# xtcyclist/hash_join_codes_KNL

Measured on AMD Instinct MI355X. Metric: probe Gtuples/s + % HBM roofline, PHJ |R|=64M join |S|=1G, 1/2/4/8 GPU, higher is better.
Workload: dtype u32

## Files before the change

### hash_join_codes_knl_amd/csrc/hj_internal.hpp

```cpp
#pragma once
#include <hip/hip_runtime.h>
#include <stdint.h>
#include <type_traits>
#include "../../include/hjgpu.h"
#include "compact_layout.hpp"

typedef unsigned long long u64;

constexpr uint32_t HJ_LINE_TUPLES = 16;
constexpr uint32_t HJ_STREAM_UNIT = 256;
constexpr uint32_t HJ_MAX_HEAVY = 128;
struct ScatterConfig { int block, vpt; bool carry; };
struct HjTuning;
ScatterConfig hj_scatter_config(const HjTuning &t, int pass, uint32_t F, bool out_packed);
int hj_scatter_tile(const HjTuning &t, int pass, uint32_t F, bool out_packed);
constexpr int HJ_JOIN_SLICE    = 1 << 16;
constexpr int HJ_JOIN_FILL_GROUPS = 64;
inline size_t hj_join_items_capacity(size_t partitions, size_t outer_rows)
{
    return (partitions + outer_rows / HJ_JOIN_SLICE + 1) * HJ_JOIN_FILL_GROUPS;
}

struct JoinConfig {
    int block, log2slots, batch;
    int slots() const { return 1 << log2slots; }
    int cap() const { return slots() / 2; }
};
const JoinConfig &hj_join_config_big();
bool hj_join_config_built(const JoinConfig &c, bool unique);

struct HjTuning {
    int range_tiles = 0;
    bool dense2 = false;
    bool npj_refhash = false;
    bool no_broadcast = false;
    bool force_chained = false;
    bool scatter_prof = false;
    bool unique = false;
    bool piece_interleave = true;
    bool merged_plan = true;
    int placement = 12;
    int placement_ms = 500;
    bool placement_log = false;
    bool exact_probe_counts = false;
    int probe_slack = 12;
    bool solo = false;
    bool audit = false;
    int hist_min_lds = 0;
    int reserve_cus = 0;
    long long host_batch = -1;
    long long group_from = 300000000, group_inner = 64000000;
    bool group_always = false;
    bool group_device = true;
    int group_slack = 50;
    long long batch_tuples = 0;
    JoinConfig join = {512, 13, 2};
    int scatter_cfg[2][3] = {{0, 0, -1}, {0, 0, -1}};
};
void hj_tuning_from_env(HjTuning *t);
bool hj_tuning_set(HjTuning *t, const char *name, const char *value);
inline const JoinConfig &hj_join_config_of(const HjTuning &t, bool big_tables) { return big_tables ? hj_join_config_big() : t.join; }

struct HjPerDeviceOnce { unsigned char done[64]; };
int hj_allow_dynamic_lds(const void *kernel, int bytes, HjPerDeviceOnce *once);

constexpr uint32_t HJ_MAX_RANGE_ENTRIES = 1u << 24;
constexpr uint32_t HJ_MAX_CHUNKS = 256;
constexpr uint32_t HJ_TICKET_K4 = 0;
constexpr uint32_t HJ_TICKET_K6 = 2 * HJ_MAX_CHUNKS;
constexpr uint32_t HJ_TICKET_MULTI_FILL = 2 * HJ_MAX_CHUNKS + 8;
constexpr uint32_t HJ_TICKET_JOIN = 2 * HJ_MAX_CHUNKS + 10;
constexpr uint32_t HJ_TICKET_JOIN2 = 2 * HJ_MAX_CHUNKS + 12;
constexpr uint32_t HJ_TICKET_JOIN3 = 2 * HJ_MAX_CHUNKS + 14;
constexpr uint32_t HJ_TICKET_WORDS = 2 * HJ_MAX_CHUNKS + 16;
struct Pass1Geom {
    u64 n, part;
#if defined(__HIPCC__)
    __host__ __device__
#endif
    u64 beg(uint32_t c) const { return c >= chunks ? n : part * c; }
    uint32_t chunks;
    uint32_t align;
    uint32_t ranges_per_chunk;
    uint32_t tile;
};
// ... 76 lines not shown
    u64 *final_offsets;
    uint32_t *overflow;
    uint32_t nt_rows;
    uint32_t big_tables;
    uint32_t broadcast;
    uint32_t mode;
    const uint32_t *sentinel;
    uint32_t force_chained;
    uint32_t unique;
    u64 *work_counter2;
    const uint32_t *multi_fill;
    uint32_t resume;
    uint32_t s_pieces;
    uint32_t *build_bits;
    u64 *work_counter3;
};
int hj_launch_build_rows(const JoinArgs &a, const HjTuning &t, int cus, hipStream_t stream);
int hj_launch_build_unmatched(const JoinArgs &a, const HjTuning &t, int cus, hipStream_t stream);

struct PlanArgs {
    const u64 *counts[2];
    u64 n[2];
    u64 chunk_beg[2][9];
    u64 *more[2] = {nullptr, nullptr};
    uint32_t regular[2];
    u64 chunk_part[2];
    u64 *off2[2];
    u64 *end2[2];
    uint32_t pad2;
    u64 *cur2[2];
// ... 46 lines not shown
int hj_launch_plan(const PlanArgs &a, hipStream_t stream);
int hj_launch_claimed_pieces(const u64 *off2, const u64 *end2, const u64 *cur2, uint32_t P, u64 *pieces_beg, u64 *pieces_end, hipStream_t stream);
int hj_launch_claimed_desc(const u64 *claim_cursors, u64 cap1, uint32_t F1, uint32_t F2, uint32_t tile2, uint4 *tdesc, uint32_t tdesc_cap,
                           u64 *total, uint32_t *overflow, hipStream_t stream);
struct BatchPlanArgs {
    const uint32_t *range_counts;
    u64 *range_base;
    u64 *boff;
    u64 *tp2b;
    uint4 *tdesc;
    uint32_t tdesc_cap;
    uint32_t ranges, ranges_per_batch, F1, F2, tile2;
};
int hj_launch_batch_plan(const BatchPlanArgs &a, uint32_t batches, hipStream_t stream);
int hj_launch_scatter(const ScatterArgs &a, const HjTuning &t, int cus, hipStream_t stream);
int hj_launch_join(const JoinArgs &a, const HjTuning &t, int cus, hipStream_t stream);
int hj_launch_exscan(const u64 *in, u64 *out, uint32_t n, hipStream_t stream);
int hj_launch_offsets_to_counts(const u64 *off, u64 *counts, uint32_t P, hipStream_t stream);

template <class F>
inline void hj_with_bool(bool b, F &&f)
{
    if (b) f(std::true_type{});
    else f(std::false_type{});
}

int hj_launch_npj_build(const uint32_t *keys, const uint32_t *vals, size_t n, u64 *table,
                        size_t buckets, uint32_t factor, uint32_t *zero_key_flag,
                        int cus, hipStream_t stream, bool line_hash = false);
struct NpjProbeArgs {
    const uint32_t *keys, *vals;
// ... 104 lines not shown
```

### hash_join_codes_knl_amd/csrc/hjgpu_api.hip

```cpp
#include "hjgpu_ctx.hpp"
#include "hj_device.hpp"

using namespace hjapi;



namespace hjapi {


int fail(hjgpu_ctx *ctx, int status, const char *what, hipError_t e)
{
    if (ctx) {
        if (e != hipSuccess)
            snprintf(ctx->err, sizeof(ctx->err), "%s: %s", what, hipGetErrorString(e));
        else
            snprintf(ctx->err, sizeof(ctx->err), "%s", what);
    }
    return status;
}

static int release(hjgpu_ctx *ctx, void *p)
{
    if (!p) return HJGPU_OK;
    HIPCHK(ctx, hipFree(p));
// ... 157 lines not shown
        m.end2[r] = take((size_t)C * P);
        m.cur2[r] = take((size_t)C * P);
        m.off1[r] = take((size_t)C * F1 + 1);
        m.cur1[r] = take((size_t)C * F1);
        m.tp1[r] = take(C + 1);
        m.seg1[r] = take(C + 1);
        m.tp2[r] = take((size_t)C * F1 + 1);
        m.seg2[r] = take((size_t)F1 + 1);
        m.more[r] = C > 8 ? take(P) : nullptr;
    }
    m.claim_total = take(1);
    m.pieces = take((size_t)4 * P);
    m.slice_prefix = take((size_t)P + 1);
    m.slices = take(P);
    m.item_part = reinterpret_cast<uint32_t *>(take(((size_t)P + items_extra + 2) / 2 + 1));
    for (int r = 0; r < 2; ++r) {
        m.range_counts[r] = reinterpret_cast<uint32_t *>(take((ranges * F1 + 1) / 2));
        m.range_base[r] = take(ranges * F1);
    }
    m.tdesc_cap = tiles2;
    for (int r = 0; r < 2; ++r) m.tdesc[r] = reinterpret_cast<uint4 *>(take(tiles2 * 4));
    m.boff = take(batches * ((size_t)F1 + 1));
    m.tp2b = take(batches * ((size_t)F1 + 1));
    m.tdescb = reinterpret_cast<uint4 *>(take(batches * tdesc_b_cap * 4));
    m.btickets = reinterpret_cast<uint32_t *>(take(batches + 1));
    m.btickets_bytes = (batches + 1) * sizeof(u64);
    m.total_bytes = at * sizeof(u64);
    return m;
}

// ... 664 lines not shown
        ja.slice_prefix = m.slice_prefix; ja.slices = m.slices; ja.item_part = m.item_part;
        ja.P = pl.P; ja.chunks = road.pad2 ? 1u : pl.C;
        ja.f1 = pl.f1; ja.F1 = pl.F1; ja.f2 = pl.f2; ja.F2 = pl.F2;
        if (o.pre) { ja.f1 = pl.pre_f1; ja.F1 = pl.pre_F1tot; ja.p1_base = pl.pre_base; }
        ja.tf0 = pl.tf0; ja.tf1 = pl.tf1;
        ja.s_align = 0;
        ja.packed = 1;
        ja.big_tables = pl.big_tables ? 1u : 0u;
        ja.unique = pl.first_match ? 1u : 0u;
        ja.mode = pl.mode;
        ja.result = &st->result;
        ja.work_counter = reinterpret_cast<u64 *>(m.tickets + HJ_TICKET_JOIN);
        ja.work_counter2 = reinterpret_cast<u64 *>(m.tickets + HJ_TICKET_JOIN2);
        ja.work_counter3 = reinterpret_cast<u64 *>(m.tickets + HJ_TICKET_JOIN3);
        ja.multi_fill = m.tickets + HJ_TICKET_MULTI_FILL;
        ja.resume = o.grp ? 1u : 0u;
        join_output(ctx, ja, o.out, bs, bl, st);
        if (marks) {
            ja.build_bits = reinterpret_cast<uint32_t *>(ctx->build_bits.p);
            HIPCHK(ctx, hj_zero_async(ja.build_bits, build_bits_bytes(pl, nn[0]), stream));
            if ((!nn[1] || build_rows) && bs && !o.grp) HIPCHK(ctx, hj_fill_async(ctx->final_offsets.p, 0xFFFFFFFFu, (size_t)workers * sizeof(u64), stream));
        }
        if (nn[1]) CHK(hj_launch_join(ja, ctx->tune, ctx->cus, stream));
        if (build_rows) CHK(hj_launch_build_rows(ja, ctx->tune, ctx->cus, stream));
        else if (marks) CHK(hj_launch_build_unmatched(ja, ctx->tune, ctx->cus, stream));
        if (audit) CHK(hj_audit_copy(reinterpret_cast<const u64 *>(&st->result), audit + 4 * 6, 4, stream));
        return HJGPU_OK;
    }
};

}

int phj_enqueue(hjgpu_ctx *ctx, const PhjPlan &pl, const Rel &R, const Rel &S, hipStream_t stream, const EnqueueOpts &o)
{
    CHK(refuse_capture(ctx, stream));
    if (o.grp && (o.pre || o.stages != PHJ_WHOLE || o.inner_ready)) return fail(ctx, HJGPU_EINVAL, "internal: a device-planned group is a whole join on resident columns");
    if ((o.pre != nullptr) != (pl.pre != 0)) return fail(ctx, HJGPU_EINVAL, "internal: plan and relations disagree about pre-partitioning");
    PhjRun run(ctx, pl, R, S, o, stream);
// ... 6 lines not shown
    CHK(run.begin());
    CHK(run.road.merged ? run.partition_merged() : run.partition_in_turn());
    if (hj_mode_marks_build(pl.mode) && (o.pre || o.stages != PHJ_WHOLE)) return fail(ctx, HJGPU_EINVAL, "internal: a join that marks its build rows is a whole join");
    if (run.road.joins) CHK(run.join(bs, bl, workers));
    record(ctx, EV_JOIN, stream);
    if (bs && run.road.joins && !o.grp) CHK(close_gaps(ctx, o.out, workers, bs, run.st, stream, pl.mode));
    record(ctx, EV_GAPS, stream);
    ctx->stats.fanout1 = pl.F1; ctx->stats.fanout2 = pl.F2; ctx->stats.buckets = 0; ctx->stats.batches = run.batches_used;
    ctx->last_algo = 1;
    return HJGPU_OK;
}

static int finish_from(hjgpu_ctx *ctx, const DevState &h, hjgpu_result *result, const hjgpu_output *out)
{
    if (result) *result = h.result;
    if (h.zero_key) return fail(ctx, HJGPU_EZEROKEY, "NPJ: a build key is 0, the empty-bucket sentinel");
    if (h.overflow) return fail(ctx, HJGPU_EOVERFLOW, "materialised output exceeded its capacity");
    if (out && out->d_keys && h.dense != h.result.count && (h.result.count != 0 || h.dense != 0))
        return fail(ctx, HJGPU_EHIP, "internal: dense length != match count after close_gaps");
    return HJGPU_OK;
}

static int read_state(hjgpu_ctx *ctx, DevState &h, hipStream_t stream)
{
    HIPCHK(ctx, hipMemcpyAsync(&h, ctx->state.p, sizeof(DevState), hipMemcpyDeviceToHost, stream));
    HIPCHK(ctx, hipStreamSynchronize(stream));
    return HJGPU_OK;
}

int finish_blocking(hjgpu_ctx *ctx, hjgpu_result *result, const hjgpu_output *out, hipStream_t stream)
// ... 303 lines not shown
        CHK(phj_prepare(ctx, cap_r, cap_s, &prm, 8, &pl, {.plan_inner = plan_inner}));
    } else {
        CHK(phj_prepare(ctx, inner, outer, &prm, 8, &pl));
        if (claimed_probe_allowed(ctx)) CHK(phj_prepare(ctx, inner, outer, &prm, 1, &pl, {.claim_s = true}));
    }
    size_t buckets; uint32_t factor;
    CHK(npj_prepare(ctx, inner, nullptr, &buckets, &factor));
    return HJGPU_OK;
}

static size_t lds_lookup_rows(const HjTuning &tune);
int hjgpu_get_counter(hjgpu_ctx *ctx, const char *name, uint64_t *value)
{
    if (!ctx || !name || !value) return HJGPU_EINVAL;
    if (strcmp(name, "probe_fallbacks") == 0) { *value = ctx->probe_fallbacks; return HJGPU_OK; }
    if (strcmp(name, "probe_exact") == 0) { *value = (ctx->tune.exact_probe_counts || ctx->probe_exact) ? 1u : 0u; return HJGPU_OK; }
    if (strcmp(name, "lookup_lds_rows") == 0) { *value = lds_lookup_rows(ctx->tune); return HJGPU_OK; }
    if (strcmp(name, "compact_ranges") == 0) { *value = hj_compact::ranges_of(ctx->cus); return HJGPU_OK; }
    if (strcmp(name, "compact_chunk_rows") == 0) { *value = hj_compact::CHUNK_ROWS; return HJGPU_OK; }
    return fail(ctx, HJGPU_EINVAL, "unknown counter (probe_fallbacks, probe_exact, lookup_lds_rows, compact_ranges, compact_chunk_rows)");
}

static void fill_reserve(const hjgpu_ctx *ctx, hjgpu_stats *s)
{
    s->ms_reserve = ctx->ms_reserve;
    s->placement_tried = ctx->placement_tried; s->placement_timeboxed = ctx->placement_timeboxed;
    s->placement_fill_ms = ctx->placement_fill_ms; s->placement_search_ms = ctx->placement_search_ms; s->placement_bytes = (uint64_t)ctx->placement_bytes;
}

int hjgpu_get_stats(hjgpu_ctx *ctx, hjgpu_stats *s)
{
    if (!ctx || !s) return HJGPU_EINVAL;
    if (ctx->stats_override) {
        *s = ctx->stats;
        fill_reserve(ctx, s);
// ... 536 lines not shown
        const Rel g_s = {g_sk + pc[g].s0, g_sv + pc[g].s0, pc[g].sn};
        if (pc[g].rn == 0) {
            CHK(broadcast_enqueue(ctx, {g_rk, g_rv, 0}, g_s, prm, vout, stream, nullptr));
        } else {
            CHK(phj_prepare(ctx, pc[g].rn, pc[g].sn, prm, chunks, &pl));
            CHK(phj_enqueue(ctx, pl, {g_rk + pc[g].r0, g_rv + pc[g].r0, pc[g].rn}, g_s, stream, {.out = vout}));
        }
        DevState h;
        CHK(read_state(ctx, h, stream));
        CHK(hjgpu_get_stats(ctx, &one));
        sum.ms_histogram += one.ms_histogram; sum.ms_plan += one.ms_plan; sum.ms_scatter1 += one.ms_scatter1;
        sum.ms_scatter2 += one.ms_scatter2; sum.ms_join += one.ms_join; sum.ms_close_gaps += one.ms_close_gaps;
        sum.fanout1 = one.fanout1; sum.fanout2 = one.fanout2;
        acc.result.count += h.result.count; acc.result.sum_keys += h.result.sum_keys;
        acc.result.sum_outer_vals += h.result.sum_outer_vals; acc.result.sum_inner_vals += h.result.sum_inner_vals;
        if (h.overflow) { acc.overflow = 1; out_on = false; }
        else if (vout) acc.dense += h.dense;
    }
    HIPCHK(ctx, hipMemcpyAsync(ctx->state.p, &acc, sizeof(DevState), hipMemcpyHostToDevice, stream));
    HIPCHK(ctx, hipStreamSynchronize(stream));
    sum.ms_total = sum.ms_scatter0 + sum.ms_histogram + sum.ms_plan + sum.ms_scatter1 + sum.ms_scatter2 + sum.ms_join + sum.ms_close_gaps;
    sum.groups = G;
    ctx->stats = sum;
    ctx->stats_override = true;
    ctx->last_algo = 1;
    return HJGPU_OK;
}

static void grouped_caps(const hjgpu_ctx *ctx, uint32_t G, size_t inner, size_t outer, size_t *cap_r, size_t *cap_s, size_t *plan_inner)
{
// ... 220 lines not shown
```

### hash_join_codes_knl_amd/csrc/hjgpu_ctx.hpp

```cpp
#pragma once
#include <hip/hip_runtime.h>
#include <algorithm>
#include <chrono>
#include <functional>
#include <math.h>
#include <stdio.h>
#include <stdlib.h>
#include <string.h>
#include <thread>
#include <vector>

#include "hj_internal.hpp"


struct DevBuf {
    void *p = nullptr;
    size_t cap = 0;
};

namespace hjapi {
struct Rel { const uint32_t *keys = nullptr, *vals = nullptr; size_t rows = 0; };
}

struct DevState {
    hjgpu_result result;
    u64 block_counter;
    u64 dense;
    u64 work_counter;
    uint32_t overflow;
    uint32_t zero_key;
    uint32_t nmoves;
    uint32_t pad;
    u64 work_counter2;
    uint32_t group_skew;
    uint32_t probe_overflow;
};

enum { EV_BEGIN = 0, EV_S_HIST, EV_S_PLAN, EV_S_SC1, EV_S_SC2, EV_WAITED,
       EV_R_HIST, EV_R_PLAN, EV_R_SC1, EV_R_SC2, EV_JOIN, EV_GAPS, EV_COUNT };


struct hjgpu_ctx {
    int device = 0;
    int cus = 0;
    hipDeviceProp_t prop;
    char err[512];
    DevBuf tmp[8];
    DevBuf meta;
    DevBuf table;
    DevBuf state;
// ... 6 lines not shown
    hjgpu_stats stats;
    int last_algo = -1;
    bool last_lookup = false;
    bool prepared = false;
    size_t prepared_inner = 0, prepared_max_outer = 0;
    unsigned char prepared_plan[128];
    HjTuning tune;
    hipStream_t host_streams[3] = {nullptr, nullptr, nullptr};
    void *host_stage[4] = {nullptr, nullptr, nullptr, nullptr};
    hipEvent_t host_stage_ev[4] = {nullptr, nullptr, nullptr, nullptr};
    hjgpu_output pending_out;
    bool has_pending_out = false;
    bool last_had_output = false;
    uint64_t probe_fallbacks = 0;
    bool probe_exact = false;
    bool rows_plain = false;
    DevBuf grp[4], grp_off;
    bool stats_override = false;
    hipStream_t aux = nullptr;
    hipEvent_t *ev_cur = nullptr;
    std::vector<hipEvent_t> grp_ev;
    uint32_t grp_ev_groups = 0;
    hipEvent_t grp_ev_pass0[3] = {nullptr, nullptr, nullptr};
    struct GroupedCall {
        bool valid = false;
        uint32_t chunks = 1;
        hjapi::Rel R, S;
        bool has_prm = false, has_out = false;
        hjgpu_phj_params prm;
        hjgpu_output out;
// ... 70 lines not shown
    return n < 1 ? 1 : n;
}

inline uint32_t align_of(const void *p) { return (uint32_t)(((uintptr_t)p >> 2) & 3); }

struct MetaLayout {
    u64 *counts[2], *off2[2], *end2[2], *cur2[2], *off1[2], *cur1[2], *tp1[2], *seg1[2], *tp2[2];
    u64 *claim1;
    u64 *claim_total;
    u64 *pieces;
    u64 *seg2[2];
    u64 *more[2];
    u64 *slice_prefix, *slices;
    uint32_t *tickets;
    uint32_t *item_part;
    uint4 *tdesc[2];
    size_t tdesc_cap;
    uint32_t *range_counts[2];
    u64 *range_base[2];
    u64 *boff, *tp2b;
    uint4 *tdescb;
    uint32_t *btickets;
    size_t btickets_bytes;
    size_t counts_bytes;
    size_t total_bytes;
};
MetaLayout carve(void *base, uint32_t C, uint32_t F1, uint32_t P, size_t ranges, size_t items_extra = 0,
                 size_t tiles2 = 0, size_t batches = 0, size_t tdesc_b_cap = 0);
ScatterArgs scatter_pass1(const hjgpu_ctx *ctx, const MetaLayout &m, int r, const Pass1Geom &geom, uint32_t F, uint32_t factor,
                          const uint32_t *kin, const uint32_t *vin, uint32_t *kout, uint32_t *vout);
// ... 92 lines not shown
```

### hash_join_codes_knl_amd/csrc/join_kernels.hip

```cpp
#include "hj_device.hpp"
#include "hj_internal.hpp"
#include "hj_emit.hpp"
#include "hj_lookup.hpp"

constexpr int hj_join_wgs_per_cu(int block, int log2slots)
{
    const int by_lds = (160 * 1024) / ((1 << log2slots) * 8 + 1024 + 9 * 1024), by_threads = 2048 / block;
    const int n = by_lds < by_threads ? by_lds : by_threads;
    return n < 1 ? 1 : n;
}
constexpr int hj_join_waves_per_simd(int block, int log2slots)
{
    const int w = hj_join_wgs_per_cu(block, log2slots) * (block / 64) / 4;
    return w < 1 ? 1 : w;
}

template <int LOG2SLOTS>
__device__ __forceinline__ uint2 hj_cuckoo_slots(uint32_t key, uint32_t tf0, uint32_t tf1)
{
    const uint32_t a1 = (key * tf0) >> (32 - LOG2SLOTS);
    return make_uint2(a1, (a1 + (((key * tf1) >> (32 - LOG2SLOTS)) | 1u)) & ((1u << LOG2SLOTS) - 1));
}

#ifndef HJ_EMIT4
// ... 3 lines not shown
    __device__ uint32_t operator()(const uint32_t (&)[4], const uint32_t (&)[4], const bool (&)[4]) const { return 0u; }
};
struct hj_mark_pass {
    __device__ uint32_t operator()(const uint32_t (&)[4], const uint32_t (&)[4], const bool (&)[4]) const { return 0u; }
};

template <bool ON, uint32_t WORDS>
struct SlotBits {
    static __device__ __forceinline__ uint32_t *get() { __shared__ uint32_t bits[WORDS]; return bits; }
};
template <uint32_t WORDS>
struct SlotBits<false, WORDS> {
    static __device__ __forceinline__ uint32_t *get() { return nullptr; }
};

template <int BLOCK, int LOG2SLOTS, int BATCH, bool PACKED, bool UNIQUE, bool DEDUP, bool NTROWS, int MODE>
__device__ __forceinline__ void join_body(JoinArgs a)
{
    constexpr bool LEFTISH = MODE == HJ_MODE_LEFT_OUTER || MODE == HJ_MODE_FULL_OUTER;
    constexpr bool MARKING = MODE == HJ_MODE_MARK;
    constexpr bool KEEPB = MODE == HJ_MODE_RIGHT_OUTER || MODE == HJ_MODE_FULL_OUTER || MARKING;
    static_assert(UNIQUE || !DEDUP || MODE == HJ_MODE_LEFT_OUTER || MARKING, "DEDUP is the multi-fill half of a _UNIQUE or left / full outer join");
    static_assert(MODE == HJ_MODE_INNER || ((UNIQUE || LEFTISH || KEEPB) && NTROWS),
                  "semi- and anti-joins walk to the first match; rows non-temporal");
    static_assert(!(KEEPB && UNIQUE), "right and full outer joins walk to every copy of a build key");
    static_assert(!(KEEPB && DEDUP) || MARKING, "the multi-fill items of a full outer join are marked by a launch of its own");
    constexpr bool SPLIT = UNIQUE || LEFTISH || MARKING;
    if (DEDUP && a.multi_fill && *a.multi_fill == 0) return;
    constexpr uint32_t SLOTS = 1u << LOG2SLOTS;
    constexpr uint32_t MASK = SLOTS - 1;
    constexpr uint32_t CAP = SLOTS / 2;
    constexpr int SHIFT = 32 - LOG2SLOTS;
    constexpr int NW = BLOCK / 64;
    constexpr int RB = 8;
    constexpr int CUCKOO_MAX_EVICTIONS = 64;
    __shared__ u64 tab64[SLOTS];
    __shared__ u64 red[4][NW];
    __shared__ u64 wave_cursor[NW];
    __shared__ uint32_t cuckoo_failed;
    constexpr uint32_t MATCHED_WORDS = (DEDUP && !MARKING) ? (HJ_JOIN_SLICE + 64) / 32 + 2 : 1;
    __shared__ uint32_t matched[MATCHED_WORDS];
    constexpr bool dedup = DEDUP;
    uint2 *tab = reinterpret_cast<uint2 *>(tab64);
// ... 421 lines not shown
                const u64 m = __ballot(hit);
                const uint32_t lane = hj_lane(), sh = (uint32_t)at & 31u;
                if (m && (sh == 0 || lane == 0)) {
                    const uint32_t w = (uint32_t)((m >> lane) << sh);
                    if (w) atomicOr(&a.build_bits[at >> 5], w);
                }
            }
            seen += len;
        }
    };

    __shared__ u64 d_item[2], d_rb[2], d_rn[2];
    __shared__ u64 d_rows_beg[2], d_rows_end[2];
    __shared__ uint32_t d_q[2], d_slice[2], d_nslices[2];
    auto claim = [&](int slot) {
        const u64 w = atomicAdd(a.work_counter, 1ull);
        d_item[slot] = w;
        if (w < total_items) {
            const uint32_t nq = a.item_part[w];
            d_q[slot] = nq;
            const u64 shape = a.slices[nq];
            const uint32_t nslices = (uint32_t)shape, groups = (uint32_t)(shape >> 32);
            const uint32_t t = (uint32_t)(w - a.slice_prefix[nq]);
            const u64 rb = a.roff[nq], rn = a.rend[nq] - rb;
            d_rb[slot] = rb;
            d_rn[slot] = rn;
            d_nslices[slot] = nslices | (a.s_pieces << 24);
            u64 rows = rn;
            for (uint32_t c = 1; c < C; ++c) rows += a.rend[(u64)c * P + nq] - a.roff[(u64)c * P + nq];
            if (groups == 1) {
                d_slice[slot] = t;
// ... 120 lines not shown
        if (rows_beg >= rows_end) __syncthreads();
        par ^= 1;
    }

    if (a.ok) hj_leave_cursor(a.final_offsets, wave_cursor);

    hj_add_to_result(red, a.result, acc_n, acc_k, acc_o, acc_i);
}

template <int BLOCK, int LOG2SLOTS, int BATCH, bool PACKED, bool UNIQUE, bool DEDUP = false, bool NTROWS = true>
__global__ __launch_bounds__(BLOCK, hj_join_waves_per_simd(BLOCK, LOG2SLOTS)) void join_kernel(JoinArgs a)
{
    join_body<BLOCK, LOG2SLOTS, BATCH, PACKED, UNIQUE, DEDUP, NTROWS, HJ_MODE_INNER>(a);
}

template <int BLOCK, int LOG2SLOTS, int BATCH, bool PACKED, int MODE, bool DEDUP>
__global__ __launch_bounds__(BLOCK, hj_join_waves_per_simd(BLOCK, LOG2SLOTS)) void exists_probe_kernel(JoinArgs a)
{
    join_body<BLOCK, LOG2SLOTS, BATCH, PACKED, true, DEDUP, true, MODE>(a);
}

template <int BLOCK, int LOG2SLOTS, int BATCH, bool PACKED, bool UNIQUE, bool DEDUP>
__global__ __launch_bounds__(BLOCK, hj_join_waves_per_simd(BLOCK, LOG2SLOTS)) void outer_probe_kernel(JoinArgs a)
{
    join_body<BLOCK, LOG2SLOTS, BATCH, PACKED, UNIQUE, DEDUP, true, HJ_MODE_LEFT_OUTER>(a);
}

template <int BLOCK, int LOG2SLOTS, int BATCH, bool PACKED>
__global__ __launch_bounds__(BLOCK, hj_join_waves_per_simd(BLOCK, LOG2SLOTS)) void right_probe_kernel(JoinArgs a)
{
// ... 274 lines not shown
int hj_launch_build_rows(const JoinArgs &a, const HjTuning &t, int cus, hipStream_t stream)
{
    if (!hj_mode_reports_build(a.mode) || !a.packed || !a.build_bits || a.P < 1 || a.chunks == 0 || (a.ok && (!a.final_offsets || !a.oiv))) return HJGPU_EINVAL;
    const JoinConfig &c = hj_join_config_of(t, a.big_tables != 0);
    const int grid = join_grid(cus, c);
    const u64 pieces = (u64)a.P * a.chunks;
    u64 split = (u64)grid * 4 / pieces;
    split = split < 1 ? 1 : split > 4096 ? 4096 : split;
    const uint32_t flip = a.mode == HJ_MODE_RIGHT_SEMI ? ~0u : 0u;
    if (c.block == 512) hipLaunchKernelGGL((build_rows_kernel<512>), dim3(grid), dim3(512), 0, stream, a, (uint32_t)split, flip);
    else if (c.block == 1024) hipLaunchKernelGGL((build_rows_kernel<1024>), dim3(grid), dim3(1024), 0, stream, a, (uint32_t)split, flip);
    else return HJGPU_EINVAL;
    return hipGetLastError() == hipSuccess ? HJGPU_OK : HJGPU_EHIP;
}

int hj_launch_join(const JoinArgs &a, const HjTuning &t, int cus, hipStream_t stream)
{
    if ((a.P < 2 && !a.broadcast) || a.P < 1 || a.chunks == 0) return HJGPU_EINVAL;
    const JoinConfig &c = hj_join_config_of(t, a.big_tables != 0);
    JoinArgs b = a;
    b.force_chained = t.force_chained ? 1u : 0u;
    b.unique = (a.unique || t.unique) ? 1u : 0u;
    if ((b.unique || b.mode) && !b.work_counter2) return HJGPU_EINVAL;
    if (hj_mode_keeps_build(b.mode) && (b.unique || !b.build_bits)) return HJGPU_EINVAL;
    if (hj_mode_reports_build(b.mode) && !b.build_bits) return HJGPU_EINVAL;
    const int grid = join_grid(cus, c);
    if (c.block == 512 && c.log2slots == 13) return launch_join_at<512, 13, true>(b, c.batch, grid, stream);
    if (c.block == 1024 && c.log2slots == 14) return launch_join_at<1024, 14, true>(b, c.batch, grid, stream);
    if (c.block == 256 && c.log2slots == 12) return launch_join_at<256, 12, false>(b, c.batch, grid, stream);
    return HJGPU_EINVAL;
}

struct LdsFill { const uint32_t *rk, *rv; uint32_t inner, tf0, tf1, force_chained; uint32_t *zero_key; };
template <int BLOCK, int LOG2SLOTS>
__device__ __forceinline__ bool lds_lookup_fill(const LdsFill &a, u64 *tab64, uint32_t &cuckoo_failed)
{
    constexpr uint32_t SLOTS = 1u << LOG2SLOTS;
// ... 187 lines not shown
```

### hash_join_codes_knl_amd/csrc/partition_kernels.hip

```cpp
#include "hj_device.hpp"
#include "hj_internal.hpp"
#include <stdlib.h>
#include <stdio.h>
#include <string.h>
#include <type_traits>

#ifndef HJ_K6_STORE
#define HJ_K6_STORE 1
#endif
__device__ __forceinline__ void k6_store16(u64 *p, uint4 v)
{
#if HJ_K6_STORE == 1 || HJ_K6_STORE == 3
    typedef uint32_t v4u_t __attribute__((ext_vector_type(4)));
    v4u_t t = {v.x, v.y, v.z, v.w};
    __builtin_nontemporal_store(t, reinterpret_cast<v4u_t *>(p));
#elif HJ_K6_STORE == 2
    __hip_atomic_store(p, (u64)v.x | ((u64)v.y << 32), __ATOMIC_RELAXED, __HIP_MEMORY_SCOPE_SYSTEM);
    __hip_atomic_store(p + 1, (u64)v.z | ((u64)v.w << 32), __ATOMIC_RELAXED, __HIP_MEMORY_SCOPE_SYSTEM);
#else
    *reinterpret_cast<uint4 *>(p) = v;
#endif
}
template <bool NT>
__device__ __forceinline__ void k6_store8(u64 *p, u64 v)
// ... 1445 lines not shown
    }
    if (is("batch_tuples")) {
        char *end = nullptr;
        const long long x = strtoll(value, &end, 10);
        if (end == value || *end) return false;
        t->batch_tuples = x;
        return true;
    }
    if (is("range_tiles")) {
        char *end = nullptr;
        const long x = strtol(value, &end, 10);
        if (end == value || *end || x < 0 || x > (1 << 20)) return false;
        t->range_tiles = (int)x;
        return true;
    }
    if (is("join_cfg")) {
        int b, l, u;
        if (!*value) { t->join = JoinConfig{512, 13, 2}; return true; }
        if (sscanf(value, "%d,%d,%d", &b, &l, &u) != 3) return false;
        t->join = JoinConfig{b, l, u};
        return true;
    }
    if (is("scatter_cfg") || is("scatter2_cfg")) {
        int *o = t->scatter_cfg[is("scatter_cfg") ? 0 : 1];
        int b, v, c = -1;
        if (!*value) { o[0] = 0; o[1] = 0; o[2] = -1; return true; }
        if (sscanf(value, "%d,%d,%d", &b, &v, &c) < 2 || b <= 0 || v <= 0) return false;
        o[0] = b; o[1] = v; o[2] = c;
        return true;
    }
    return false;
}

void hj_tuning_from_env(HjTuning *t)
{
    static const char *const names[] = {"dense2", "npj_refhash", "no_broadcast", "force_chained", "scatter_prof",
                                        "unique", "merged_plan", "piece_interleave", "range_tiles", "batch_tuples", "group_from", "group_inner", "group_always", "group_device", "group_slack", "host_batch", "placement", "placement_ms", "placement_log", "audit", "solo", "exact_probe_counts", "probe_slack", "hist_min_lds", "reserve_cus", "join_cfg", "scatter_cfg", "scatter2_cfg"};
    for (const char *n : names) {
        char env[64] = "HJGPU_";
        size_t at = strlen(env);
        for (const char *c = n; *c && at + 1 < sizeof(env); ++c) env[at++] = (char)((*c >= 'a' && *c <= 'z') ? *c - 32 : *c);
        env[at] = 0;
        const char *v = getenv(env);
        if (v && *v && !hj_tuning_set(t, n, v))
            fprintf(stderr, "hjgpu: ignoring malformed %s=%s\n", env, v);
    }
}
```

Baseline: 124.6.

## Add lean aggregate-only inner join kernel with deferred fallback list

Adds a specialised inner-join kernel for the packed, single-chunk, non-unique, count/sum-only case. It builds a cuckoo table in LDS, probes four keys per vector load and reduces the aggregates in registers, with optional prefetching of the next item's build rows. Partitions that overflow the LDS capacity or fail cuckoo insertion are appended to a deferred item list, which a second, listed launch of the general join kernel then processes. This removes the general kernel's per-item overhead on the common path, at the cost of an extra launch, atomic list appends and a second code path to keep correct.

```diff
diff --git a/hash_join_codes_knl_amd/csrc/hj_internal.hpp b/hash_join_codes_knl_amd/csrc/hj_internal.hpp
--- a/hash_join_codes_knl_amd/csrc/hj_internal.hpp
+++ b/hash_join_codes_knl_amd/csrc/hj_internal.hpp
@@ -28,6 +28,8 @@
 };
 const JoinConfig &hj_join_config_big();
 bool hj_join_config_built(const JoinConfig &c, bool unique);
+struct JoinAggConfig { int block, batch, prefetch; };
+bool hj_join_agg_config(int block, int batch, int prefetch, JoinAggConfig *out);
 
 struct HjTuning {
     int range_tiles = 0;
@@ -55,6 +57,8 @@
     int group_slack = 50;
     long long batch_tuples = 0;
     JoinConfig join = {512, 13, 2};
+    bool lean_join = true;
+    JoinAggConfig lean_cfg = {1024, 1, 1};
     int scatter_cfg[2][3] = {{0, 0, -1}, {0, 0, -1}};
 };
 void hj_tuning_from_env(HjTuning *t);
@@ -69,6 +73,7 @@
 constexpr uint32_t HJ_TICKET_K4 = 0;
 constexpr uint32_t HJ_TICKET_K6 = 2 * HJ_MAX_CHUNKS;
 constexpr uint32_t HJ_TICKET_MULTI_FILL = 2 * HJ_MAX_CHUNKS + 8;
+constexpr uint32_t HJ_TICKET_DEFERRED = 2 * HJ_MAX_CHUNKS + 9;
 constexpr uint32_t HJ_TICKET_JOIN = 2 * HJ_MAX_CHUNKS + 10;
 constexpr uint32_t HJ_TICKET_JOIN2 = 2 * HJ_MAX_CHUNKS + 12;
 constexpr uint32_t HJ_TICKET_JOIN3 = 2 * HJ_MAX_CHUNKS + 14;
@@ -175,6 +180,9 @@
     uint32_t s_pieces;
     uint32_t *build_bits;
     u64 *work_counter3;
+    uint32_t *item_list;
+    uint32_t *item_count;
+    uint32_t *lean_deferred;
 };
 int hj_launch_build_rows(const JoinArgs &a, const HjTuning &t, int cus, hipStream_t stream);
 int hj_launch_build_unmatched(const JoinArgs &a, const HjTuning &t, int cus, hipStream_t stream);
@@ -251,7 +259,7 @@
 };
 int hj_launch_batch_plan(const BatchPlanArgs &a, uint32_t batches, hipStream_t stream);
 int hj_launch_scatter(const ScatterArgs &a, const HjTuning &t, int cus, hipStream_t stream);
-int hj_launch_join(const JoinArgs &a, const HjTuning &t, int cus, hipStream_t stream);
+int hj_launch_join(const JoinArgs &a, const HjTuning &t, int cus, hipStream_t stream, bool *lean = nullptr);
 int hj_launch_exscan(const u64 *in, u64 *out, uint32_t n, hipStream_t stream);
 int hj_launch_offsets_to_counts(const u64 *off, u64 *counts, uint32_t P, hipStream_t stream);
 
diff --git a/hash_join_codes_knl_amd/csrc/hjgpu_api.hip b/hash_join_codes_knl_amd/csrc/hjgpu_api.hip
--- a/hash_join_codes_knl_amd/csrc/hjgpu_api.hip
+++ b/hash_join_codes_knl_amd/csrc/hjgpu_api.hip
@@ -195,6 +195,7 @@
     m.slice_prefix = take((size_t)P + 1);
     m.slices = take(P);
     m.item_part = reinterpret_cast<uint32_t *>(take(((size_t)P + items_extra + 2) / 2 + 1));
+    m.item_list = reinterpret_cast<uint32_t *>(take(((size_t)P + items_extra + 2) / 2 + 1));
     for (int r = 0; r < 2; ++r) {
         m.range_counts[r] = reinterpret_cast<uint32_t *>(take((ranges * F1 + 1) / 2));
         m.range_base[r] = take(ranges * F1);
@@ -889,6 +890,7 @@
         ja.work_counter2 = reinterpret_cast<u64 *>(m.tickets + HJ_TICKET_JOIN2);
         ja.work_counter3 = reinterpret_cast<u64 *>(m.tickets + HJ_TICKET_JOIN3);
         ja.multi_fill = m.tickets + HJ_TICKET_MULTI_FILL;
+        ja.item_list = m.item_list; ja.item_count = m.tickets + HJ_TICKET_DEFERRED; ja.lean_deferred = &st->lean_deferred;
         ja.resume = o.grp ? 1u : 0u;
         join_output(ctx, ja, o.out, bs, bl, st);
         if (marks) {
@@ -896,7 +898,9 @@
             HIPCHK(ctx, hj_zero_async(ja.build_bits, build_bits_bytes(pl, nn[0]), stream));
             if ((!nn[1] || build_rows) && bs && !o.grp) HIPCHK(ctx, hj_fill_async(ctx->final_offsets.p, 0xFFFFFFFFu, (size_t)workers * sizeof(u64), stream));
         }
-        if (nn[1]) CHK(hj_launch_join(ja, ctx->tune, ctx->cus, stream));
+        bool lean = false;
+        if (nn[1]) CHK(hj_launch_join(ja, ctx->tune, ctx->cus, stream, &lean));
+        if (lean) ++ctx->lean_joins;
         if (build_rows) CHK(hj_launch_build_rows(ja, ctx->tune, ctx->cus, stream));
         else if (marks) CHK(hj_launch_build_unmatched(ja, ctx->tune, ctx->cus, stream));
         if (audit) CHK(hj_audit_copy(reinterpret_cast<const u64 *>(&st->result), audit + 4 * 6, 4, stream));
@@ -933,6 +937,7 @@
 static int finish_from(hjgpu_ctx *ctx, const DevState &h, hjgpu_result *result, const hjgpu_output *out)
 {
     if (result) *result = h.result;
+    ctx->lean_deferred_items += h.lean_deferred;
     if (h.zero_key) return fail(ctx, HJGPU_EZEROKEY, "NPJ: a build key is 0, the empty-bucket sentinel");
     if (h.overflow) return fail(ctx, HJGPU_EOVERFLOW, "materialised output exceeded its capacity");
     if (out && out->d_keys && h.dense != h.result.count && (h.result.count != 0 || h.dense != 0))
@@ -1266,11 +1271,13 @@
 {
     if (!ctx || !name || !value) return HJGPU_EINVAL;
     if (strcmp(name, "probe_fallbacks") == 0) { *value = ctx->probe_fallbacks; return HJGPU_OK; }
+    if (strcmp(name, "lean_joins") == 0) { *value = ctx->lean_joins; return HJGPU_OK; }
+    if (strcmp(name, "lean_deferred_items") == 0) { *value = ctx->lean_deferred_items; return HJGPU_OK; }
     if (strcmp(name, "probe_exact") == 0) { *value = (ctx->tune.exact_probe_counts || ctx->probe_exact) ? 1u : 0u; return HJGPU_OK; }
     if (strcmp(name, "lookup_lds_rows") == 0) { *value = lds_lookup_rows(ctx->tune); return HJGPU_OK; }
     if (strcmp(name, "compact_ranges") == 0) { *value = hj_compact::ranges_of(ctx->cus); return HJGPU_OK; }
     if (strcmp(name, "compact_chunk_rows") == 0) { *value = hj_compact::CHUNK_ROWS; return HJGPU_OK; }
-    return fail(ctx, HJGPU_EINVAL, "unknown counter (probe_fallbacks, probe_exact, lookup_lds_rows, compact_ranges, compact_chunk_rows)");
+    return fail(ctx, HJGPU_EINVAL, "unknown counter (probe_fallbacks, probe_exact, lean_joins, lean_deferred_items, lookup_lds_rows, compact_ranges, compact_chunk_rows)");
 }
 
 static void fill_reserve(const hjgpu_ctx *ctx, hjgpu_stats *s)
@@ -1837,6 +1844,7 @@
         sum.fanout1 = one.fanout1; sum.fanout2 = one.fanout2;
         acc.result.count += h.result.count; acc.result.sum_keys += h.result.sum_keys;
         acc.result.sum_outer_vals += h.result.sum_outer_vals; acc.result.sum_inner_vals += h.result.sum_inner_vals;
+        acc.lean_deferred += h.lean_deferred;
         if (h.overflow) { acc.overflow = 1; out_on = false; }
         else if (vout) acc.dense += h.dense;
     }
diff --git a/hash_join_codes_knl_amd/csrc/hjgpu_ctx.hpp b/hash_join_codes_knl_amd/csrc/hjgpu_ctx.hpp
--- a/hash_join_codes_knl_amd/csrc/hjgpu_ctx.hpp
+++ b/hash_join_codes_knl_amd/csrc/hjgpu_ctx.hpp
@@ -34,6 +34,8 @@
     u64 work_counter2;
     uint32_t group_skew;
     uint32_t probe_overflow;
+    uint32_t lean_deferred;
+    uint32_t pad2;
 };
 
 enum { EV_BEGIN = 0, EV_S_HIST, EV_S_PLAN, EV_S_SC1, EV_S_SC2, EV_WAITED,
@@ -70,6 +72,7 @@
     bool last_had_output = false;
     uint64_t probe_fallbacks = 0;
     bool probe_exact = false;
+    uint64_t lean_joins = 0, lean_deferred_items = 0;
     bool rows_plain = false;
     DevBuf grp[4], grp_off;
     bool stats_override = false;
@@ -170,6 +173,7 @@
     u64 *slice_prefix, *slices;
     uint32_t *tickets;
     uint32_t *item_part;
+    uint32_t *item_list;
     uint4 *tdesc[2];
     size_t tdesc_cap;
     uint32_t *range_counts[2];
diff --git a/hash_join_codes_knl_amd/csrc/join_kernels.hip b/hash_join_codes_knl_amd/csrc/join_kernels.hip
--- a/hash_join_codes_knl_amd/csrc/join_kernels.hip
+++ b/hash_join_codes_knl_amd/csrc/join_kernels.hip
@@ -41,7 +41,7 @@
     static __device__ __forceinline__ uint32_t *get() { return nullptr; }
 };
 
-template <int BLOCK, int LOG2SLOTS, int BATCH, bool PACKED, bool UNIQUE, bool DEDUP, bool NTROWS, int MODE>
+template <int BLOCK, int LOG2SLOTS, int BATCH, bool PACKED, bool UNIQUE, bool DEDUP, bool NTROWS, int MODE, bool LISTED = false>
 __device__ __forceinline__ void join_body(JoinArgs a)
 {
     constexpr bool LEFTISH = MODE == HJ_MODE_LEFT_OUTER || MODE == HJ_MODE_FULL_OUTER;
@@ -54,6 +54,7 @@
     static_assert(!(KEEPB && DEDUP) || MARKING, "the multi-fill items of a full outer join are marked by a launch of its own");
     constexpr bool SPLIT = UNIQUE || LEFTISH || MARKING;
     if (DEDUP && a.multi_fill && *a.multi_fill == 0) return;
+    if (LISTED && *a.item_count == 0) return;
     constexpr uint32_t SLOTS = 1u << LOG2SLOTS;
     constexpr uint32_t MASK = SLOTS - 1;
     constexpr uint32_t CAP = SLOTS / 2;
@@ -505,7 +506,8 @@
     __shared__ u64 d_rows_beg[2], d_rows_end[2];
     __shared__ uint32_t d_q[2], d_slice[2], d_nslices[2];
     auto claim = [&](int slot) {
-        const u64 w = atomicAdd(a.work_counter, 1ull);
+        u64 w = atomicAdd(a.work_counter, 1ull);
+        if constexpr (LISTED) w = w < *a.item_count ? (u64)a.item_list[w] : total_items;
         d_item[slot] = w;
         if (w < total_items) {
             const uint32_t nq = a.item_part[w];
@@ -656,6 +658,218 @@
     join_body<BLOCK, LOG2SLOTS, BATCH, PACKED, UNIQUE, DEDUP, NTROWS, HJ_MODE_INNER>(a);
 }
 
+template <int BLOCK, int LOG2SLOTS, int BATCH>
+__global__ __launch_bounds__(BLOCK, hj_join_waves_per_simd(BLOCK, LOG2SLOTS)) void join_listed_kernel(JoinArgs a)
+{
+    join_body<BLOCK, LOG2SLOTS, BATCH, true, false, false, true, HJ_MODE_INNER, true>(a);
+}
+
+constexpr int hj_join_agg_wgs_per_cu(int block, int log2slots)
+{
+    const int by_lds = (160 * 1024) / ((1 << log2slots) * 8 + 1024), by_threads = 2048 / block;
+    const int n = by_lds < by_threads ? by_lds : by_threads;
+    return n < 1 ? 1 : n;
+}
+constexpr int hj_join_agg_waves_per_simd(int block, int log2slots)
+{
+    const int w = hj_join_agg_wgs_per_cu(block, log2slots) * (block / 64) / 4;
+    return w < 1 ? 1 : w;
+}
+
+template <int BLOCK, int LOG2SLOTS, int BATCH, bool PREFETCH>
+__global__ __launch_bounds__(BLOCK, hj_join_agg_waves_per_simd(BLOCK, LOG2SLOTS)) void join_agg_kernel(JoinArgs a)
+{
+    constexpr uint32_t SLOTS = 1u << LOG2SLOTS;
+    constexpr uint32_t CAP = SLOTS / 2;
+    constexpr int SHIFT = 32 - LOG2SLOTS;
+    constexpr int NW = BLOCK / 64;
+    constexpr int RB = (int)((CAP + BLOCK - 1) / BLOCK);
+    constexpr int CUCKOO_MAX_EVICTIONS = 64;
+    __shared__ u64 tab64[SLOTS];
+    __shared__ u64 red[4][NW];
+    __shared__ uint32_t cuckoo_failed;
+    __shared__ u64 d_item[2], d_rb[2];
+    __shared__ uint32_t d_rn[2], d_q[2], d_slice[2], d_nslices[2];
+
+    uint32_t tid = threadIdx.x;
+    const uint32_t P = a.P;
+    const u64 total_items = a.slice_prefix[P];
+    const uint4 *__restrict__ sk4 = reinterpret_cast<const uint4 *>(a.sk);
+    const u64 *__restrict__ r64 = reinterpret_cast<const u64 *>(a.rk);
+    const uint32_t tf0 = a.tf0, tf1 = a.tf1;
+    u64 acc_n = 0, acc_k = 0, acc_o = 0, acc_i = 0;
+
+    auto defer = [&](u64 w) {
+        const uint32_t at = atomicAdd(a.item_count, 1u);
+        hj_store(&a.item_list[at], (uint32_t)w);
+        atomicAdd(a.lean_deferred, 1u);
+    };
+    auto claim = [&](int slot) {
+        const u64 w = atomicAdd(a.work_counter, 1ull);
+        d_item[slot] = w;
+        if (w < total_items) {
+            const uint32_t nq = a.item_part[w];
+            const u64 shape = a.slices[nq];
+            const uint32_t nslices = (uint32_t)shape, groups = (uint32_t)(shape >> 32);
+            const uint32_t t = (uint32_t)(w - a.slice_prefix[nq]);
+            const u64 rb = a.roff[nq], rows = a.rend[nq] - rb;
+            u64 beg = 0, end = rows;
+            uint32_t slice = t;
+            if (groups != 1) {
+                const uint32_t group = t / nslices;
+                slice = t - group * nslices;
+                const uint32_t fills = (uint32_t)((rows + CAP - 1) >> (LOG2SLOTS - 1));
+                const uint32_t per_group = (fills + groups - 1) / groups;
+                beg = min(rows, (u64)group * per_group * CAP);
+                end = min(rows, (u64)(group + 1) * per_group * CAP);
+            }
+            const bool left = end - beg > CAP || (a.force_chained && end > beg);
+            if (left) defer(w);
+            d_q[slot] = nq;
+            d_slice[slot] = slice;
+            d_nslices[slot] = nslices | (a.s_pieces << 24);
+            d_rb[slot] = rb + beg;
+            d_rn[slot] = left ? 0u : (uint32_t)(end - beg);
+        }
+    };
+    uint32_t pk[RB], pv[RB];
+#pragma unroll
+    for (int j = 0; j < RB; ++j) { pk[j] = 0; pv[j] = 0; }
+    auto load_rows = [&](int slot, uint32_t lane_tid) {
+        const u64 *__restrict__ rows = r64 + hj_uniform(d_rb[slot]);
+        const uint32_t n = hj_uniform(d_item[slot]) < total_items ? hj_uniform(d_rn[slot]) : 0u;
+#pragma unroll
+        for (int j = 0; j < RB; ++j) {
+            const uint32_t i = (uint32_t)j * BLOCK + lane_tid;
+            pk[j] = 0; pv[j] = 0;
+            if (i < n) { const u64 t = rows[i]; pk[j] = (uint32_t)t; pv[j] = (uint32_t)(t >> 32); }
+        }
+    };
+
+    int par = 0;
+    if (tid == 0) claim(0);
+    __syncthreads();
+    if (PREFETCH) load_rows(0, tid);
+    for (;;) {
+        const u64 w = hj_uniform(d_item[par]);
+        if (w >= total_items) break;
+        const uint32_t q = hj_uniform(d_q[par]);
+        const u64 slice = hj_uniform(d_slice[par]);
+        const uint32_t nslices_word = hj_uniform(d_nslices[par]);
+        const uint32_t rn = hj_uniform(d_rn[par]);
+        if (tid == 0) claim(par ^ 1);
+        asm volatile("" : "+v"(tid));
+        const uint32_t ltid = tid;
+        if (rn == 0) {
+            __syncthreads();
+            if (PREFETCH) load_rows(par ^ 1, ltid);
+            par ^= 1;
+            continue;
+        }
+        uint32_t empty = 0;
+        while ((hj_hash(empty, a.f1, a.F1) - a.p1_base) * a.F2 + hj_hash(empty, a.f2, a.F2) == q) ++empty;
+        const u64 EMPTY64 = (u64)empty;
+
+        uint32_t h0 = tf0, h1 = tf1;
+        if (!PREFETCH) load_rows(par, ltid);
+        constexpr int TRIES = 4;
+#pragma unroll 1
+        for (int attempt = 1;; ++attempt) {
+            for (uint32_t i = ltid; i < SLOTS; i += BLOCK) tab64[i] = EMPTY64;
+            if (tid == 0) cuckoo_failed = 0;
+            __syncthreads();
+#pragma unroll
+            for (int j = 0; j < RB; ++j) {
+                if ((uint32_t)j * BLOCK + ltid >= rn) continue;
+                u64 cur = (u64)pk[j] | ((u64)pv[j] << 32);
+                uint32_t loc = (pk[j] * h0) >> SHIFT;
+                int it = 0;
+                for (; it < CUCKOO_MAX_EVICTIONS; ++it) {
+                    const u64 old = atomicExch(&tab64[loc], cur);
+                    if ((uint32_t)old == empty) break;
+                    const uint2 a12 = hj_cuckoo_slots<LOG2SLOTS>((uint32_t)old, h0, h1);
+                    loc = (loc == a12.x) ? a12.y : a12.x;
+                    cur = old;
+                    if (it >= 8 && cuckoo_failed) it = CUCKOO_MAX_EVICTIONS - 1;
+                }
+                if (it == CUCKOO_MAX_EVICTIONS) cuckoo_failed = 1;
+            }
+            __syncthreads();
+            if (!hj_uniform(cuckoo_failed) || attempt == TRIES) break;
+            h0 = (h0 * 0x9E3779B1u) | 1u; h1 = (h1 * 0x85EBCA6Bu) | 1u;
+            __syncthreads();
+        }
+        if (PREFETCH) load_rows(par ^ 1, ltid);
+        if (hj_uniform(cuckoo_failed)) {
+            if (tid == 0) defer(w);
+        } else {
+            const u64 nslices = nslices_word & 0xFFFFFFu;
+            const uint32_t pieces = 1u + (nslices_word >> 24);
+            for (uint32_t c = 0; c < pieces; ++c) {
+                const u64 b = a.soff[(u64)c * P + q], e = a.send[(u64)c * P + q];
+                const u64 len = e - b;
+                if (len == 0) continue;
+                const u64 gb = b + (len * slice) / nslices;
+                const u64 ge = b + (len * (slice + 1)) / nslices;
+                for (u64 run = gb & ~3ull; run < ge; run += 1ull << 24) {
+                    const uint4 *__restrict__ s4 = sk4 + (run >> 1);
+                    const uint32_t lo = gb > run ? (uint32_t)(gb - run) : 0u;
+                    const uint32_t hi = (uint32_t)min(ge - run, (u64)1 << 24);
+                    for (uint32_t r0 = ltid * 4; r0 < hi; r0 += (uint32_t)BLOCK * 4 * BATCH) {
+                        uint4 kk[BATCH], vv[BATCH];
+#pragma unroll
+                        for (int u = 0; u < BATCH; ++u) {
+                            const uint32_t r = r0 + (uint32_t)u * BLOCK * 4;
+                            kk[u] = make_uint4(0, 0, 0, 0); vv[u] = kk[u];
+                            if (r < hi) { kk[u] = s4[r >> 1]; vv[u] = s4[(r >> 1) + 1]; }
+                        }
+#pragma unroll
+                        for (int u = 0; u < BATCH; ++u) {
+                            const uint32_t r = r0 + (uint32_t)u * BLOCK * 4;
+                            if (r >= hi) break;
+                            const uint32_t key[4] = {kk[u].x, kk[u].z, vv[u].x, vv[u].z};
+                            const uint32_t val[4] = {kk[u].y, kk[u].w, vv[u].y, vv[u].w};
+                            u64 t1[4], t2[4];
+#pragma unroll
+                            for (int j = 0; j < 4; ++j) {
+                                const uint2 at = hj_cuckoo_slots<LOG2SLOTS>(key[j], h0, h1);
+                                t1[j] = tab64[at.x];
+                                t2[j] = tab64[at.y];
+                            }
+                            u64 sk_ = 0, so_ = 0, si_ = 0;
+                            uint32_t n = 0;
+#pragma unroll
+                            for (int j = 0; j < 4; ++j) {
+                                const bool valid = (r + j >= lo) && (r + j < hi);
+                                const bool h1 = valid && ((uint32_t)t1[j] == key[j]);
+                                const bool h2 = valid && ((uint32_t)t2[j] == key[j]);
+                                const uint32_t m = (h1 ? 1u : 0u) + (h2 ? 1u : 0u);
+                                n += m;
+                                sk_ += (u64)key[j] * m;
+                                so_ += (u64)val[j] * m;
+                                si_ += (h1 ? (uint32_t)(t1[j] >> 32) : 0u);
+                                si_ += (h2 ? (uint32_t)(t2[j] >> 32) : 0u);
+                            }
+                            acc_n += n; acc_k += sk_; acc_o += so_; acc_i += si_;
+                        }
+                    }
+                }
+            }
+        }
+        __syncthreads();
+        par ^= 1;
+    }
+    acc_n = wave_reduce_sum(acc_n); acc_k = wave_reduce_sum(acc_k);
+    acc_o = wave_reduce_sum(acc_o); acc_i = wave_reduce_sum(acc_i);
+    if ((tid & 63u) == 0) { red[0][tid >> 6] = acc_n; red[1][tid >> 6] = acc_k; red[2][tid >> 6] = acc_o; red[3][tid >> 6] = acc_i; }
+    __syncthreads();
+    if (tid < 4) {
+        u64 s = 0;
+        for (int i = 0; i < NW; ++i) s += red[tid][i];
+        if (s) atomicAdd(reinterpret_cast<u64 *>(a.result) + tid, s);
+    }
+}
+
 template <int BLOCK, int LOG2SLOTS, int BATCH, bool PACKED, int MODE, bool DEDUP>
 __global__ __launch_bounds__(BLOCK, hj_join_waves_per_simd(BLOCK, LOG2SLOTS)) void exists_probe_kernel(JoinArgs a)
 {
@@ -960,13 +1174,42 @@
     return hipGetLastError() == hipSuccess ? HJGPU_OK : HJGPU_EHIP;
 }
 
-int hj_launch_join(const JoinArgs &a, const HjTuning &t, int cus, hipStream_t stream)
-{
+#define HJ_JOIN_AGG_BUILT(X) X(768, 2, false) X(768, 1, true) X(640, 2, true) X(1024, 1, true) X(1024, 1, false)
+bool hj_join_agg_config(int block, int batch, int prefetch, JoinAggConfig *out)
+{
+#define X(B, U, PF) if (block == B && (batch < 0 || (batch == U && (prefetch != 0) == PF))) { if (out) *out = JoinAggConfig{B, U, PF ? 1 : 0}; return true; }
+    HJ_JOIN_AGG_BUILT(X)
+#undef X
+    return false;
+}
+
+static int launch_join_agg(const JoinArgs &b, const JoinAggConfig &g, int cus, hipStream_t stream)
+{
+    JoinKernel lean = nullptr;
+#define X(B, U, PF) if (g.block == B && g.batch == U && (g.prefetch != 0) == PF) lean = join_agg_kernel<B, 13, U, PF>;
+    HJ_JOIN_AGG_BUILT(X)
+#undef X
+    if (!lean) return HJGPU_EINVAL;
+    hipLaunchKernelGGL(lean, dim3(cus * hj_join_agg_wgs_per_cu(g.block, 13)), dim3(g.block), 0, stream, b);
+    JoinArgs d = b;
+    d.work_counter = b.work_counter2;
+    hipLaunchKernelGGL((join_listed_kernel<512, 13, 2>), dim3(cus * hj_join_wgs_per_cu(512, 13)), dim3(512), 0, stream, d);
+    return hipGetLastError() == hipSuccess ? HJGPU_OK : HJGPU_EHIP;
+}
+
+int hj_launch_join(const JoinArgs &a, const HjTuning &t, int cus, hipStream_t stream, bool *lean)
+{
+    if (lean) *lean = false;
     if ((a.P < 2 && !a.broadcast) || a.P < 1 || a.chunks == 0) return HJGPU_EINVAL;
     const JoinConfig &c = hj_join_config_of(t, a.big_tables != 0);
     JoinArgs b = a;
     b.force_chained = t.force_chained ? 1u : 0u;
     b.unique = (a.unique || t.unique) ? 1u : 0u;
+    if (t.lean_join && b.mode == HJ_MODE_INNER && !b.ok && b.packed && b.chunks == 1 && !b.unique && !b.broadcast && !b.big_tables &&
+        c.block == 512 && c.log2slots == 13 && c.batch == 2 && b.item_list && b.item_count && b.lean_deferred && b.work_counter2) {
+        if (lean) *lean = true;
+        return launch_join_agg(b, t.lean_cfg, cus, stream);
+    }
     if ((b.unique || b.mode) && !b.work_counter2) return HJGPU_EINVAL;
     if (hj_mode_keeps_build(b.mode) && (b.unique || !b.build_bits)) return HJGPU_EINVAL;
     if (hj_mode_reports_build(b.mode) && !b.build_bits) return HJGPU_EINVAL;
diff --git a/hash_join_codes_knl_amd/csrc/partition_kernels.hip b/hash_join_codes_knl_amd/csrc/partition_kernels.hip
--- a/hash_join_codes_knl_amd/csrc/partition_kernels.hip
+++ b/hash_join_codes_knl_amd/csrc/partition_kernels.hip
@@ -1483,6 +1483,14 @@
         t->range_tiles = (int)x;
         return true;
     }
+    if (is("lean_join")) return parse_flag(value, &t->lean_join);
+    if (is("lean_join_cfg")) {
+        int b = 0, u = -1, pf = 0;
+        if (!*value) { t->lean_cfg = HjTuning().lean_cfg; return true; }
+        const int n = sscanf(value, "%d,%d,%d", &b, &u, &pf);
+        if (n != 1 && n != 3) return false;
+        return hj_join_agg_config(b, n == 1 ? -1 : u, pf, &t->lean_cfg);
+    }
     if (is("join_cfg")) {
         int b, l, u;
         if (!*value) { t->join = JoinConfig{512, 13, 2}; return true; }
@@ -1504,7 +1512,7 @@
 void hj_tuning_from_env(HjTuning *t)
 {
     static const char *const names[] = {"dense2", "npj_refhash", "no_broadcast", "force_chained", "scatter_prof",
-                                        "unique", "merged_plan", "piece_interleave", "range_tiles", "batch_tuples", "group_from", "group_inner", "group_always", "group_device", "group_slack", "host_batch", "placement", "placement_ms", "placement_log", "audit", "solo", "exact_probe_counts", "probe_slack", "hist_min_lds", "reserve_cus", "join_cfg", "scatter_cfg", "scatter2_cfg"};
+                                        "unique", "merged_plan", "piece_interleave", "range_tiles", "batch_tuples", "group_from", "group_inner", "group_always", "group_device", "group_slack", "host_batch", "placement", "placement_ms", "placement_log", "audit", "solo", "exact_probe_counts", "probe_slack", "hist_min_lds", "reserve_cus", "join_cfg", "lean_join", "lean_join_cfg", "scatter_cfg", "scatter2_cfg"};
     for (const char *n : names) {
         char env[64] = "HJGPU_";
         size_t at = strlen(env);
```

After: 125.5, median of 3. Within noise of the previous version (+0.7%).
